# trevordblack/Physically_Based_Renderer

Hardware: AMD Instinct MI355X
Metric: shaded pixels/sec (Mpix/s) + achieved HBM GB/s, 4K G-buffer, 64 lights (higher is better)
Workload: dtype f32

## Files before the change

physically_based_renderer_amd/csrc/pbr_balanced.h:

```cpp
#pragma once
#include <cstdint>
#include <type_traits>

#include "pbr_device_math.h"
#include "pbr_device_math_x2.h"
#include "shade_kernels.h"

namespace pbr {

constexpr int kBalRec = 7;

#ifndef PBR_BAL_PROFILE
#define PBR_BAL_PROFILE 0
#endif
#if PBR_BAL_PROFILE
__device__ unsigned long long* g_bal_prof_buf;
#define BAL_PROF_T(v) const long long v = (long long)__builtin_amdgcn_s_memtime()
#define BAL_PROF_ADD(slot_, val_) do { if ((threadIdx.x & 63) == 0) bal_prof[slot_] += (unsigned long long)(val_); } while (0)
#else
#define BAL_PROF_T(v)
#define BAL_PROF_ADD(i, x)
#endif

constexpr int kBalLdsStride = kBalMaxLights + 4;
// ... 357 lines not shown
                    lz = lds_lights[2 * kBalLdsStride + lane_id];
        const float b0 = ((fabsf(lx - cx) + fabsf(ly - cy)) + fabsf(lz - cz)) + slack;
        const float fr = ((fabsf(lx) + fabsf(ly)) + fabsf(lz)) + pmax;
        bj = (b0 + 0.125f * fr) * (1.0f + 0x1p-20f);
        const float fx = fmaxf(fabsf(lx - mnx), fabsf(lx - mxx)), fy = fmaxf(fabsf(ly - mny), fabsf(ly - mxy)),
                    fz = fmaxf(fabsf(lz - mnz), fabsf(lz - mxz));
        const float gx = fmaxf(fmaxf(mnx - lx, lx - mxx), 0.0f), gy = fmaxf(fmaxf(mny - ly, ly - mxy), 0.0f),
                    gz = fmaxf(fmaxf(mnz - lz, lz - mxz), 0.0f);
        near = (fx * fx + fy * fy) + fz * fz <= 99.9f * 99.9f;
        far = (gx * gx + gy * gy) + gz * gz >= 100.1f * 100.1f;
        close = !((gx * gx + gy * gy) + gz * gz >= (1.02f * dist_lo) * (1.02f * dist_lo));
    }
    const float bmax = bal_wave_max<F>(bj);
    const uint64_t far_m = lanes(far), cross_m = lanes(!near && !far), close_m = lanes(close);
    const v2 cn = v2{0x1p-18f * ((fabsf(n.x.x) + fabsf(n.y.x)) + fabsf(n.z.x)),
                     0x1p-18f * ((fabsf(n.x.y) + fabsf(n.y.y)) + fabsf(n.z.y))};
    const v2 nd = -vfma(n.z, pos.z, vfma(n.y, pos.y, n.x * pos.x));
    const v2 kb = vfma(cn, splat(bmax), nd);
    uint32_t a0 = 0, a1 = 0, c0 = 0, c1 = 0;
    typedef __attribute__((address_space(3))) const float lds_float;
    const uint32_t lbase = (uint32_t)(uintptr_t)(const lds_float*)lds_lights;
    auto word = [&](int qbase, uint32_t& ma, uint32_t& mb) {
        for (int k = 6; k >= 0; k -= 2) {
            const uint32_t la = lbase + 16u * (uint32_t)(qbase + k);
            float4 x1, y1, z1, x0, y0, z0;
            asm volatile(
                "ds_read_b128 %0, %6 offset:16\n\t"
                "ds_read_b128 %1, %6 offset:288\n\t"
                "ds_read_b128 %2, %6 offset:560\n\t"
                "ds_read_b128 %3, %6\n\t"
                "ds_read_b128 %4, %6 offset:272\n\t"
                "ds_read_b128 %5, %6 offset:544\n\t"
                "s_waitcnt lgkmcnt(0)"
                : "=&v"(x1), "=&v"(y1), "=&v"(z1), "=&v"(x0), "=&v"(y0), "=&v"(z0)
                : "v"(la)
                : "memory");
            push_skip_bits4(ma, mb, x1, y1, z1, n, kb);
            push_skip_bits4(ma, mb, x0, y0, z0, n, kb);
        }
    };
    const int n0 = nl < 32 ? nl : 32;
    if (nl > 32) word(8, a1, c1);
    word(0, a0, c0);
    const int n1 = nl - n0;
    const uint32_t k0 = (n0 == 32 ? ~0u : (1u << n0) - 1u) & ~(uint32_t)far_m,
                   k1 = (n1 == 32 ? ~0u : (1u << n1) - 1u) & ~(uint32_t)(far_m >> 32);
    a0 = live_a ? ~a0 & k0 : 0u;
    c0 = live_b ? ~c0 & k0 : 0u;
    a1 = live_a ? ~a1 & k1 : 0u;
    c1 = live_b ? ~c1 & k1 : 0u;
    for (uint64_t cm = cross_m; cm != 0; cm &= cm - 1) {
        const int j = __builtin_ctzll(cm);
        const m2 out = beyond_range(pos, lds_lights[j], lds_lights[kBalLdsStride + j], lds_lights[2 * kBalLdsStride + j]);
        const uint32_t bit = 1u << (j & 31);
        const uint32_t oa = on(out.x) ? bit : 0u, ob = on(out.y) ? bit : 0u;
        if (j < 32) {
            a0 &= ~oa;
            c0 &= ~ob;
        } else {
            a1 &= ~oa;
            c1 &= ~ob;
        }
    }
    bool near_a = false, near_b = false;
    for (uint64_t cm = close_m; cm != 0; cm &= cm - 1) {
        const int j = __builtin_ctzll(cm);
        const f3x2 l = f3x2{splat(lds_lights[j]) - pos.x, splat(lds_lights[kBalLdsStride + j]) - pos.y,
                            splat(lds_lights[2 * kBalLdsStride + j]) - pos.z};
        const m2 ok = ge(sqrt_nr(dot3(l, l)), dist_lo);
        const uint32_t bit = 1u << (j & 31);
        near_a = near_a || (((j < 32 ? a0 : a1) & bit) != 0 && !on(ok.x));
        near_b = near_b || (((j < 32 ? c0 : c1) & bit) != 0 && !on(ok.y));
    }

    BAL_PROF_T(t1);
    BAL_PROF_ADD(0, t1 - t0);
    return BalMasks{a0, a1, c0, c1, near_a, near_b};
}

__device__ __forceinline__ int wave_live_items(const BalMasks& bm) {
    return wave_sum_dpp((__popc(bm.a0) + __popc(bm.a1)) + (__popc(bm.c0) + __popc(bm.c1)));
}


template <bool EXACT>
__device__ __forceinline__ void lighting_balanced_points(const PixelInvariants2& q, const Faithful2& fi,
                                                         const f3x2& pos, bool live_a, bool live_b, BalMasks bm,
                                                         BalancedWaveLds& w, const float* lds_lights, f3x2& sum,
                                                         m2& redo, unsigned long long* bal_prof = nullptr) {
    const int lane_id = (int)(threadIdx.x & 63);
    const uint32_t a0 = bm.a0, a1 = bm.a1, c0 = bm.c0, c1 = bm.c1;
    redo |= mask2(bm.near_a, bm.near_b);
    constexpr int R = EXACT ? kBalRecX : kBalRec;
    BAL_PROF_T(t1);
    PBR_PHASE("rank");

    const int cnt_a = __popc(a0) + __popc(a1), cnt_b = __popc(c0) + __popc(c1);
    w.hist[lane_id] = 0;
    wave_lds_sync();
    const int bin_a = cnt_a < 63 ? cnt_a : 63, bin_b = cnt_b < 63 ? cnt_b : 63;
    const int pos_a = atomicAdd(&w.hist[bin_a], 1);
    const int pos_b = atomicAdd(&w.hist[bin_b], 1);
    wave_lds_sync();
    const int h = w.hist[lane_id];
    const int incl = wave_scan_add_dpp(h);
    wave_lds_sync();
    w.hist[lane_id] = incl - h;
    wave_lds_sync();
    const int rank_a = w.hist[bin_a] + pos_a, rank_b = w.hist[bin_b] + pos_b;
    wave_lds_sync();
    w.rank[lane_id] = make_int2(rank_a, rank_b);
    using Item = std::conditional_t<EXACT, ItemPixelX, ItemPixel>;
    Item ia, ib;
    if constexpr (EXACT) {
        ia = item_pixel_x(q, pos, 0, a0, a1, 2 * lane_id);
        ib = item_pixel_x(q, pos, 1, c0, c1, 2 * lane_id + 1);
    } else {
        ia = item_pixel(q, fi, pos, 0, a0, a1, 2 * lane_id);
        ib = item_pixel(q, fi, pos, 1, c0, c1, 2 * lane_id + 1);
    }
    if (rank_a < 64) store_item(&w.rec[R * rank_a], ia);
    if (rank_b < 64) store_item(&w.rec[R * rank_b], ib);
    wave_lds_sync();
    Item cur = load_item_any<EXACT>(&w.rec[R * lane_id]);
    wave_lds_sync();
    if (rank_a >= 64) store_item(&w.rec[R * (127 - rank_a)], ia);
    if (rank_b >= 64) store_item(&w.rec[R * (127 - rank_b)], ib);
    wave_lds_sync();

    BAL_PROF_T(t2);
    PBR_PHASE("pass2");
    f3x2 acc = splat3(0.0f, 0.0f, 0.0f);
    f3 accx = mk3(0.0f, 0.0f, 0.0f);
    uint64_t fail = 0, second = 0;
    uint64_t m = ((uint64_t)cur.live1 << 32) | cur.live0;
    auto result = [&]() {
        const f3 r = EXACT ? accx : mk3(acc.x.x + acc.x.y, acc.y.x + acc.y.y, acc.z.x + acc.z.y);
        return make_float4(r.x, r.y, r.z, on(fail) ? 0.0f : 1.0f);
    };
    const uint32_t slot_addr = lds_addr(&w.rec[R * lane_id]);
    auto put_result = [&](int k, float4 v) {
        if (k == 0) {
            lds_write2<0>(slot_addr, v.x, v.y);
            lds_write2<2>(slot_addr, v.z, v.w);
        } else {
            lds_write2<4>(slot_addr, v.x, v.y);
            lds_write2<6>(slot_addr, v.z, v.w);
        }
    };
    auto next_pixel = [&]() {
        cur = load_item_any<EXACT>(&w.rec[R * lane_id]);
        m = ((uint64_t)cur.live1 << 32) | cur.live0;
        put_result(0, result());
        acc = splat3(0.0f, 0.0f, 0.0f);
        accx = mk3(0.0f, 0.0f, 0.0f);
    };
    uint64_t zero = lanes(m == 0);
    if (zero != 0) {
        if (on(zero)) next_pixel();
        second = zero;
        const uint64_t first_done = zero;
        zero = lanes(m == 0);
        const uint64_t empty = first_done & zero;
        if (empty != 0 && on(empty)) put_result(1, result());
    }
#if PBR_BAL_PROFILE
    int iters = 0;
#endif
    {
        const uint64_t exec = __builtin_amdgcn_read_exec();
        uint64_t live = ~zero & exec;
        while (live != 0) {
// ... 63 lines not shown
```

physically_based_renderer_amd/csrc/shade_kernels.hip:

```cpp
#include <hip/hip_runtime.h>

#include <cstdint>
#include <type_traits>
#include <vector>

#include "pbr_device_math.h"
#include "pbr_device_math_x2.h"
#include "pbr_balanced.h"
#include "shade_kernels.h"

namespace pbr {

#ifndef PBR_WAVE_TIMELINE
#define PBR_WAVE_TIMELINE 0
#endif
#if PBR_WAVE_TIMELINE
constexpr int kTlWords = 8;
static __device__ unsigned long long* g_wave_tl;
static __device__ long long g_wave_tl_cap;
#define TL_RT(i_) (tl[i_] = (unsigned long long)__builtin_amdgcn_s_memrealtime())
#define TL_BEGIN()                                                                                           \
    unsigned long long tl[kTlWords];                                                                         \
    TL_RT(1);                                                                                                \
    tl[6] = (unsigned long long)__builtin_amdgcn_s_memtime();                                                \
// ... 120 lines not shown
        off += (w < wave) ? c : 0;
        total += c;
    }
    if (keep) {
        const int slot = off + before;
        s.light[3 * slot + 0] = l0;
        s.light[3 * slot + 1] = l1;
        s.light[3 * slot + 2] = l2;
    }
    return total;
}

struct LightRec {
    float4 s, d, p;
};
__device__ __forceinline__ LightRec light_rec(const float4* __restrict__ lights, int j, const PassArgs& ps) {
    j = PBR_BOUNDS(j, ps.n_dir + ps.n_point + ps.n_spot, kBoundsLight);
    return LightRec{lights[3 * j], lights[3 * j + 1], lights[3 * j + 2]};
}
__device__ __forceinline__ m2 light_flag(const LightRec& r) {
    const uint64_t m = (__float_as_uint(r.p.w) << 1) != 0u ? ~0ull : 0ull;
    return m2{m, m};
}
__device__ __forceinline__ float uniform_f(float x) {
    return __builtin_bit_cast(float, __builtin_amdgcn_readfirstlane(__builtin_bit_cast(int, x)));
}

__device__ __forceinline__ bool light_survives(float4 lp, const TileBounds& wb) {
    const float dx = hmax(hmax(wb.mn[0] - lp.x, lp.x - wb.mx[0]), 0.0f);
    const float dy = hmax(hmax(wb.mn[1] - lp.y, lp.y - wb.mx[1]), 0.0f);
    const float dz = hmax(hmax(wb.mn[2] - lp.z, lp.z - wb.mx[2]), 0.0f);
    return (dx * dx + dy * dy + dz * dz) <= kCullRadius * kCullRadius;
}

__device__ __forceinline__ void survivor_masks(const float4* __restrict__ lights, int base, int b1,
                                               const TileBounds& wb, bool cull_enabled, uint64_t (&m)[4]) {
    const int lane = (int)(threadIdx.x & 63);
    float4 lp[4];
#pragma unroll
    for (int k = 0; k < 4; ++k) {
        const int j = base + 64 * k + lane;
        lp[k] = j < b1 && cull_enabled ? lights[3 * j + 2] : make_float4(0.0f, 0.0f, 0.0f, 0.0f);
    }
#pragma unroll
    for (int k = 0; k < 4; ++k) {
        const int j = base + 64 * k + lane;
        m[k] = lanes(j < b1 && (!cull_enabled || light_survives(lp[k], wb)));
    }
}

struct FirstSurvivors {
    uint64_t m[4];
    bool valid = false;
};
__device__ __forceinline__ int wave_light_terms(const float4* __restrict__ lights, const PassArgs& ps,
                                                const TileBounds& wb, bool cull_enabled,
                                                FirstSurvivors* first = nullptr) {
    const int b0 = ps.n_dir, b1 = ps.n_dir + ps.n_point + ps.n_spot;
    if (!cull_enabled) return b1;
    int total = ps.n_dir;
    for (int base = b0; base < b1; base += 256) {
        uint64_t m[4];
        if (first != nullptr && first->valid && base == b0) {
            for (int k = 0; k < 4; ++k) m[k] = first->m[k];
        } else {
            survivor_masks(lights, base, b1, wb, true, m);
            if (first != nullptr && base == b0 && ps.n_spot == 0) {
                for (int k = 0; k < 4; ++k) first->m[k] = m[k];
                first->valid = true;
            }
        }
        total += __popcll(m[0]) + __popcll(m[1]) + __popcll(m[2]) + __popcll(m[3]);
    }
    return total;
}

template <bool CULL, bool LEAN, bool FAITHFUL = false, bool BALANCED = false>
__device__ __forceinline__ f3x2 lighting_fast(const PixelInvariants2& q, const f3x2& pos, m2 fast_ok,
                                              const float4* __restrict__ lights, const PassArgs& ps,
                                              const TileBounds& wb, bool cull_enabled, m2& redo, int& kept_total,
                                              BalancedWaveLds* bal = nullptr, const float* bal_lights = nullptr,
                                              bool geo_a = false, bool geo_b = false, BalMasks bm = BalMasks{},
                                              unsigned long long* bal_prof = nullptr,
                                              const FirstSurvivors* first = nullptr) {
    f3x2 direct = splat3(0.0f, 0.0f, 0.0f);
    Faithful2 fi{};
    if (FAITHFUL) fi = make_faithful<!CULL>(q);
    const int n_dir = BALANCED && !FAITHFUL ? 0 : ps.n_dir;
    for (int j = 0; j < n_dir; ++j) {
        PBR_COLD("directional");
        const LightRec r = light_rec(lights, j, ps);
        m2 ok = fast_ok & light_flag(r);
        if (FAITHFUL) {
            directional_faithful_x2<LEAN, !CULL>(q, fi, r.s, r.d, ok, direct);
        } else {
            const f3x2 c = directional_x2<LEAN>(q, r.s, r.d, ok);
            direct = add3(direct, c);
        }
        redo |= ~ok;
    }
    const int pt_begin = ps.n_dir, sp_begin = ps.n_dir + ps.n_point, end = sp_begin + ps.n_spot;
    auto run_kind = [&](auto spot_tag, int b0, int b1) {
        constexpr bool SPOT = decltype(spot_tag)::value;
        auto point = [&](int j) {
            const LightRec r = light_rec(lights, j, ps);
            m2 ok = fast_ok & light_flag(r);
            if (FAITHFUL) {
                point_or_spot_faithful_x2<SPOT, LEAN, !CULL>(q, fi, pos, r.s, r.d, r.p, ok, direct);
            } else {
                const f3x2 c = point_or_spot_x2<SPOT, LEAN>(q, pos, r.s, r.d, r.p, ok);
                direct = add3(direct, c);
            }
            redo |= ~ok;
        };
        if (!CULL) {
            for (int j = b0; j < b1; ++j) point(j);
            return;
        }
        for (int base = b0; base < b1; base += 256) {
            uint64_t ms[4];
            if (!SPOT && first != nullptr && first->valid && base == b0) {
                for (int k = 0; k < 4; ++k) ms[k] = first->m[k];
            } else {
                survivor_masks(lights, base, b1, wb, cull_enabled, ms);
            }
#pragma unroll
            for (int k = 0; k < 4; ++k) {
                uint64_t m = ms[k];
                kept_total += __popcll(m);
                while (m) {
                    const int jl = base + 64 * k + __builtin_ctzll(m);
                    m &= m - 1;
                    point(jl);
                }
            }
        }
    };
    if (BALANCED)
        lighting_balanced_points<!FAITHFUL>(q, fi, pos, geo_a, geo_b, bm, *bal, bal_lights, direct, redo, bal_prof);
    else
        run_kind(std::false_type{}, pt_begin, sp_begin);
    if (!BALANCED && end > sp_begin) run_kind(std::true_type{}, sp_begin, end);
    if (FAITHFUL) {
        const m2 in_x = eq(direct.x, 0.0f) | (ge(direct.x, 0x1p-100f) & le(direct.x, 0x1p100f));
        const m2 in_y = eq(direct.y, 0.0f) | (ge(direct.y, 0x1p-100f) & le(direct.y, 0x1p100f));
        const m2 in_z = eq(direct.z, 0.0f) | (ge(direct.z, 0x1p-100f) & le(direct.z, 0x1p100f));
        redo |= ~(in_x & in_y & in_z);
    }
    return direct;
}

template <bool CULL>
__device__ __forceinline__ void lighting_exact(const PixelInvariants& qa, const PixelInvariants& qb, f3 pa, f3 pb,
                                               bool need_a, bool need_b, const float4* __restrict__ lights,
                                               const PassArgs& ps, Lds& s, const TileBounds& tb,
                                               bool cull_enabled, f3& da, f3& db) {
    da = mk3(0.0f, 0.0f, 0.0f);
    db = mk3(0.0f, 0.0f, 0.0f);
    bool unused = true;
    for (int base = 0; base < ps.n_dir; base += kChunk) {
        const int cnt = min(kChunk, ps.n_dir - base);
        __syncthreads();
        stage_chunk<false>(lights, base, cnt, s, tb, false, true);
        __syncthreads();
        for (int j = 0; j < cnt; ++j) {
            const float4* r = &s.light[3 * j];
            if (need_a) da = add3(da, directional_light<false>(qa, r[0], r[1], unused));
            if (need_b) db = add3(db, directional_light<false>(qb, r[0], r[1], unused));
        }
    }
    const int pt_begin = ps.n_dir, sp_begin = ps.n_dir + ps.n_point, end = sp_begin + ps.n_spot;
#pragma unroll 1
    for (int kind = 1; kind <= 2; ++kind) {
        const int b0 = kind == 1 ? pt_begin : sp_begin, b1 = kind == 1 ? sp_begin : end;
        for (int base = b0; base < b1; base += kChunk) {
            const int cnt = min(kChunk, b1 - base);
            __syncthreads();
            const int kept = stage_chunk<CULL>(lights, base, cnt, s, tb, cull_enabled, false);
            __syncthreads();
            for (int j = 0; j < kept; ++j) {
                const float4* r = &s.light[3 * j];
                f3 c;
                if (need_a) {
                    const bool lit = kind == 1 ? point_or_spot_light<false, false>(qa, pa, r[0], r[1], r[2], c, unused)
                                               : point_or_spot_light<true, false>(qa, pa, r[0], r[1], r[2], c, unused);
                    if (lit) da = add3(da, c);
                }
                if (need_b) {
                    const bool lit = kind == 1 ? point_or_spot_light<false, false>(qb, pb, r[0], r[1], r[2], c, unused)
                                               : point_or_spot_light<true, false>(qb, pb, r[0], r[1], r[2], c, unused);
                    if (lit) db = add3(db, c);
                }
            }
        }
    }
}

__device__ __forceinline__ void lighting_exact_wave(const PixelInvariants& qa, const PixelInvariants& qb, f3 pa,
                                                    f3 pb, bool need_a, bool need_b, const float4* __restrict__ lights,
                                                    const PassArgs& ps, f3& da, f3& db) {
    da = mk3(0.0f, 0.0f, 0.0f);
    db = mk3(0.0f, 0.0f, 0.0f);
    bool unused = true;
    for (int j = 0; j < ps.n_dir; ++j) {
        const LightRec r = light_rec(lights, j, ps);
        if (need_a) da = add3(da, directional_light<false>(qa, r.s, r.d, unused));
        if (need_b) db = add3(db, directional_light<false>(qb, r.s, r.d, unused));
    }
    const int pt_begin = ps.n_dir, sp_begin = ps.n_dir + ps.n_point, end = sp_begin + ps.n_spot;
    for (int j = pt_begin; j < end; ++j) {
        const LightRec r = light_rec(lights, j, ps);
        const bool spot = j >= sp_begin;
        f3 c;
        if (need_a) {
            const bool lit = spot ? point_or_spot_light<true, false>(qa, pa, r.s, r.d, r.p, c, unused)
                                  : point_or_spot_light<false, false>(qa, pa, r.s, r.d, r.p, c, unused);
            if (lit) da = add3(da, c);
        }
        if (need_b) {
            const bool lit = spot ? point_or_spot_light<true, false>(qb, pb, r.s, r.d, r.p, c, unused)
                                  : point_or_spot_light<false, false>(qb, pb, r.s, r.d, r.p, c, unused);
            if (lit) db = add3(db, c);
// ... 293 lines not shown
            }
        }
        const int cnt = min(64, n - base);
        for (int k = 0; k < cnt; ++k) {
            sum.x = sum.x + __builtin_bit_cast(float, __builtin_amdgcn_readlane(__builtin_bit_cast(int, t.x), k));
            sum.y = sum.y + __builtin_bit_cast(float, __builtin_amdgcn_readlane(__builtin_bit_cast(int, t.y), k));
            sum.z = sum.z + __builtin_bit_cast(float, __builtin_amdgcn_readlane(__builtin_bit_cast(int, t.z), k));
        }
    }
    return sum;
}

template <int AMBIENT, bool F0_PLANE, bool APPLY_AO, bool LANES>
__device__ __forceinline__ float4 shade_pixel_exact(const GBufferArgs& gb, const PassArgs& ps,
                                                    const float4* __restrict__ lights, const float4* __restrict__ env,
                                                    int64_t idx, bool need, bool faithful_finish) {
    if (!LANES) idx = need ? idx : 0;
    idx = PBR_BOUNDS_PIXEL(idx, gb.width, gb.height, gb.row_stride, 1, kBoundsGBuffer);
    const f3 pos = mk3(gb.plane[0][idx], gb.plane[1][idx], gb.plane[2][idx]);
    const f3 n = mk3(gb.plane[3][idx], gb.plane[4][idx], gb.plane[5][idx]);
    const f3 albedo = mk3(gb.plane[6][idx], gb.plane[7][idx], gb.plane[8][idx]);
    const float metallic = gb.plane[9][idx], roughness = gb.plane[10][idx];
    const float ao = APPLY_AO ? gb.plane[11][idx] : 1.0f;
    const f3 f0 = F0_PLANE ? mk3(gb.plane[12][idx], gb.plane[13][idx], gb.plane[14][idx])
                           : mk3(ps.fresnel_r0[0] + metallic * (albedo.x - ps.fresnel_r0[0]),
                                 ps.fresnel_r0[1] + metallic * (albedo.y - ps.fresnel_r0[1]),
                                 ps.fresnel_r0[2] + metallic * (albedo.z - ps.fresnel_r0[2]));
    const f3 eye = mk3(ps.eye[0], ps.eye[1], ps.eye[2]);
    const PixelInvariants q = make_invariants(n, normalize3(sub3(eye, pos)), albedo, f0, metallic, roughness);
    f3 d, unused;
    if (LANES)
        d = lighting_exact_lanes(q, pos, lights, ps);
    else
        lighting_exact_wave(q, q, pos, pos, need, false, lights, ps, d, unused);
    return finish_pixel<AMBIENT, APPLY_AO>(q, ao, d, ps, env, false, faithful_finish);
}

constexpr int kLanesRepassMax = 8;

template <int AMBIENT, bool F0_PLANE, bool APPLY_AO>
__device__ __forceinline__ void repass_exact(const GBufferArgs& gb, const PassArgs& ps,
                                             const float4* __restrict__ lights, const float4* __restrict__ env,
                                             const FrameArgs& fr, int tile_x, int tile_y, int wave_id, bool need_a,
                                             bool need_b, int n_exact, bool faithful) {
    const int tid = threadIdx.x & 63;
    if (n_exact <= kLanesRepassMax) {
        uint64_t ma = lanes(need_a), mb = lanes(need_b);
        while ((ma | mb) != 0) {
            const bool second = ma == 0;
            uint64_t& m = second ? mb : ma;
            const int l = __builtin_ctzll(m);
            m &= m - 1;
            const int rx = tile_x * kTileW + 2 * (l & 31) + (second ? 1 : 0);
            const int ry = tile_y * kTileH + 2 * wave_id + (l >> 5);
            float4 c = shade_pixel_exact<AMBIENT, F0_PLANE, APPLY_AO, true>(gb, ps, lights, env,
                                                                            (int64_t)ry * gb.row_stride + rx, true,
                                                                            faithful);
            if (tid == 0 && alpha_keep(gb, (int64_t)ry * gb.row_stride + rx, c))
                store_pixel(fr, (int64_t)ry * fr.out_stride + rx, c);
        }
    } else {
        const int ln = lane_id_fresh();
        const int rx = tile_x * kTileW + 2 * (ln & 31);
        const int ry = tile_y * kTileH + 2 * wave_id + (ln >> 5);
        const int64_t gi = (int64_t)ry * gb.row_stride + rx, oi = (int64_t)ry * fr.out_stride + rx;
        if (lanes(need_a) != 0) {
            float4 c = shade_pixel_exact<AMBIENT, F0_PLANE, APPLY_AO, false>(gb, ps, lights, env, gi, need_a, faithful);
            if (need_a && alpha_keep(gb, gi, c)) store_pixel(fr, oi, c);
        }
        if (lanes(need_b) != 0) {
            float4 c = shade_pixel_exact<AMBIENT, F0_PLANE, APPLY_AO, false>(gb, ps, lights, env, gi + 1, need_b,
                                                                             faithful);
            if (need_b && alpha_keep(gb, gi + 1, c)) store_pixel(fr, oi + 1, c);
        }
    }
}

template <int AMBIENT, bool F0_PLANE, bool APPLY_AO, bool CULL, int BAL = 0>
__global__ __launch_bounds__(BAL != 0 && PBR_BAL_WAVES == 1 ? 64 : kBlock, PBR_X2_MIN_WAVES) void shade_tile_kernel(
    GBufferArgs gb, PassArgs ps, const float4* __restrict__ lights, const float4* __restrict__ env, FrameArgs fr,
    int32_t* __restrict__ tile_kept, bool exact_only) {
    constexpr bool kOneWave = BAL != 0 && PBR_BAL_WAVES == 1;
    __shared__ std::conditional_t<kOneWave, LdsBal1, Lds> s;
    TL_BEGIN();
    PBR_PHASE("entry");
#if PBR_BAL_PROFILE
    const long long t_entry = (long long)__builtin_amdgcn_s_memtime();
    unsigned long long* bal_prof = s.prof[__builtin_amdgcn_readfirstlane(threadIdx.x) >> 6];
    if ((threadIdx.x & 63) < 16) bal_prof[threadIdx.x & 63] = 0;
#endif
    load_libm_tables<AMBIENT == kAmbientIblDiffuse, (BAL != 0 && PBR_BAL_WAVES == 1 ? 64 : kBlock)>();
    if constexpr (BAL != 0)
        stage_balanced_lights<kOneWave ? 64 : kBlock>(lights, ps.n_dir, ps.n_dir + ps.n_point, s.bal_light,
                                                      BAL == 2 ? 4.0f : 1.0f);
    __syncthreads();
    PBR_PHASE("load_window");

    const int wave_id = kOneWave ? (int)(blockIdx.y & 3) : __builtin_amdgcn_readfirstlane((int)threadIdx.x) >> 6;
    const int wslot = kOneWave ? 0 : wave_id;
    const int tile_y = kOneWave ? (int)(blockIdx.y >> 2) : (int)blockIdx.y;
    const int tid = kOneWave ? 64 * wave_id + (int)threadIdx.x : (int)threadIdx.x;
    const int xa = blockIdx.x * kTileW + 2 * (tid & 31);
    const int y = tile_y * kTileH + (tid >> 5);
    const bool va = (xa < gb.width) && (y < gb.height);
    const bool vb = (xa + 1 < gb.width) && (y < gb.height);
    const int64_t row = (int64_t)y * gb.row_stride;
    const bool ga = va && is_geometry(fr, xa, y), gb_ = vb && is_geometry(fr, xa + 1, y);
    const bool wave_geometry = lanes(ga || gb_) != 0;

    PairIn p = load_pair<F0_PLANE, APPLY_AO>(gb, ps, va ? row + xa : 0, vb ? row + xa + 1 : 0,
                                             vb && gb.pairs_aligned);
    const f3 pa = lane(p.pos, 0), pb = lane(p.pos, 1);

    const bool ok_a = !exact_only && ps.eye_ok && fast_window_ok(pa, lane(p.n, 0), lane(p.albedo, 0), lane(p.f0, 0),
                                                    p.metallic.x, p.roughness.x);
    const bool ok_b = !exact_only && ps.eye_ok && fast_window_ok(pb, lane(p.n, 1), lane(p.albedo, 1), lane(p.f0, 1),
                                                    p.metallic.y, p.roughness.y);
    const m2 fast2 = mask2(ok_a, ok_b);
    TL_LOADED();

    PixelInvariants2 q2;
    if constexpr (BAL == 0) q2 = pair_invariants(p, ps, fast2);
    auto form_q2 = [&]() {
        if constexpr (BAL != 0) q2 = pair_invariants(p, ps, fast2);
    };

    TileBounds wb{};
    bool cull_enabled = false;
    if (CULL) {
        const bool finite = (!ga || (isfinite(pa.x) && isfinite(pa.y) && isfinite(pa.z))) &&
                            (!gb_ || (isfinite(pb.x) && isfinite(pb.y) && isfinite(pb.z)));
        const float big = 3.0e38f;
        wb.mn[0] = uniform_f(wave_min(fminf(ga ? pa.x : big, gb_ ? pb.x : big)));
        wb.mn[1] = uniform_f(wave_min(fminf(ga ? pa.y : big, gb_ ? pb.y : big)));
        wb.mn[2] = uniform_f(wave_min(fminf(ga ? pa.z : big, gb_ ? pb.z : big)));
        wb.mx[0] = uniform_f(wave_max(fmaxf(ga ? pa.x : -big, gb_ ? pb.x : -big)));
        wb.mx[1] = uniform_f(wave_max(fmaxf(ga ? pa.y : -big, gb_ ? pb.y : -big)));
        wb.mx[2] = uniform_f(wave_max(fmaxf(ga ? pa.z : -big, gb_ ? pb.z : -big)));
        cull_enabled = lanes(!finite) == 0;
    }

    int kept_total = 0;
    int bal_items = -1;
    m2 redo = m2{0, 0};
    f3x2 pos2 = p.pos;
    f3x2 d2 = splat3(0.0f, 0.0f, 0.0f);
    bool faithful_wave = false;
    TL_RT(3);
    if (wave_geometry) {
        const v2 nn = dot3(p.n, p.n);
        const bool lean_lane = ok_a && ok_b && nn.x <= 1.0f + 0x1p-20f && nn.y <= 1.0f + 0x1p-20f &&
                               f0_nonzero(lane(p.f0, 0)) && f0_nonzero(lane(p.f0, 1));
        const bool faithful_lane =
            ps.faithful && ok_a && ok_b && p.albedo.x.x >= 0.0f && p.albedo.y.x >= 0.0f && p.albedo.z.x >= 0.0f &&
            p.albedo.x.y >= 0.0f && p.albedo.y.y >= 0.0f && p.albedo.z.y >= 0.0f && p.f0.x.x <= 1.0f &&
            p.f0.y.x <= 1.0f && p.f0.z.x <= 1.0f && p.f0.x.y <= 1.0f && p.f0.y.y <= 1.0f && p.f0.z.y <= 1.0f &&
            p.f0.x.x >= 0.0f && p.f0.y.x >= 0.0f && p.f0.z.x >= 0.0f && p.f0.x.y >= 0.0f && p.f0.y.y >= 0.0f &&
            p.f0.z.y >= 0.0f;
        faithful_wave = BAL != 2 && ps.faithful && lanes(!faithful_lane) == 0;
        if (CULL && faithful_wave && ps.faithful == 2)
            faithful_wave = wave_light_terms(lights, ps, wb, cull_enabled) <= kFaithfulMaxTerms;
        const bool lean_wave = lanes(!lean_lane) == 0;
        if (faithful_wave && lean_wave) {
            if constexpr (BAL == 1 && !CULL) {
#if PBR_BAL_PROFILE
                BAL_PROF_ADD(7, (long long)__builtin_amdgcn_s_memtime() - t_entry);
                unsigned long long* prof = s.prof[wslot];
#else
                unsigned long long* prof = nullptr;
#endif
                PBR_PHASE("pass1");
                const BalMasks bm = balanced_pass1<false>(p.pos, p.n, ga, gb_, ps.n_point, kBalDistLoFaithful, s.bal[wslot],
                                                   s.bal_light, prof);
                bal_items = wave_live_items(bm);
                PBR_PHASE("invariants");
                launder(p);
                q2 = pair_invariants(p, ps, fast2);
                faithful_scale(q2);
                d2 = lighting_fast<false, true, true, true>(q2, p.pos, fast2, lights, ps, wb, cull_enabled, redo,
                                                            kept_total, &s.bal[wslot], s.bal_light, ga, gb_, bm,
                                                            prof);
#if PBR_BAL_PROFILE
                const long long t_l1 = (long long)__builtin_amdgcn_s_memtime();
#endif
                PBR_PHASE("invariants2");
                launder(p);
                q2 = pair_finish_invariants(p, ps, fast2);
                pos2 = p.pos;
#if PBR_BAL_PROFILE
                const v2 dep = dot3(q2.n, q2.v);
                if (dep.x == 12345.0f) pos2.x.x = 0.5f;
                BAL_PROF_ADD(8, (long long)__builtin_amdgcn_s_memtime() - t_l1);
#endif
            } else {
                form_q2();
                if (!CULL) faithful_scale(q2);
#if PBR_BAL_PROFILE
                const long long t_u0 = (long long)__builtin_amdgcn_s_memtime();
                BAL_PROF_ADD(11, t_u0 - t_entry);
                BAL_PROF_ADD(13, 1);
#endif
                d2 = lighting_fast<CULL, true, true>(q2, pos2, fast2, lights, ps, wb, cull_enabled, redo, kept_total);
                if (!CULL) faithful_unscale(q2);
#if PBR_BAL_PROFILE
                const v2 dep = d2.x + d2.y;
                if (dep.x == 12345.0f) pos2.x.x = 0.5f;
                BAL_PROF_ADD(12, (long long)__builtin_amdgcn_s_memtime() - t_u0);
#endif
            }
        } else if (faithful_wave) {
            PBR_COLD("faithful_nonlean");
            form_q2();
            if (!CULL) faithful_scale(q2);
            d2 = lighting_fast<CULL, false, true>(q2, pos2, fast2, lights, ps, wb, cull_enabled, redo, kept_total);
            if (!CULL) faithful_unscale(q2);
        } else if (lean_wave) {
            PBR_PHASE("xpass1");
            if constexpr (BAL == 2 && !CULL) {
#if PBR_BAL_PROFILE
                unsigned long long* prof = s.prof[wslot];
#else
                unsigned long long* prof = nullptr;
#endif
                auto reload = [&]() {
                    asm volatile("" ::: "memory");
                    const int rl = lane_id_fresh();
                    const int rx = blockIdx.x * kTileW + 2 * (rl & 31);
                    const int ry = tile_y * kTileH + 2 * wave_id + (rl >> 5);
                    const int64_t rrow = (int64_t)ry * gb.row_stride + rx;
                    p = load_pair<F0_PLANE, APPLY_AO>(gb, ps, va ? rrow : 0, vb ? rrow + 1 : 0,
                                                      vb && gb.pairs_aligned);
                };
                const BalMasks bm = balanced_pass1<true>(p.pos, p.n, ga, gb_, ps.n_point, kBalDistLoExact, s.bal[wslot],
                                                   s.bal_light, prof);
                bal_items = wave_live_items(bm);
                PBR_PHASE("xinvariants");
                q2 = pair_invariants(p, ps, fast2);
                d2 = lighting_fast<false, true, false, true>(q2, p.pos, fast2, lights, ps, wb, cull_enabled, redo,
                                                             kept_total, &s.bal[wslot], s.bal_light, ga, gb_, bm,
                                                             prof);
                PBR_PHASE("xinvariants2");
                reload();
                q2 = pair_invariants(p, ps, fast2);
                pos2 = p.pos;
            } else {
                form_q2();
                d2 = lighting_fast<CULL, true>(q2, pos2, fast2, lights, ps, wb, cull_enabled, redo, kept_total);
            }
        } else {
            PBR_COLD("general");
            form_q2();
            d2 = lighting_fast<CULL, false>(q2, pos2, fast2, lights, ps, wb, cull_enabled, redo, kept_total);
        }
    } else {
        PBR_COLD("background");
        form_q2();
    }
    TL_RT(4);
    const PixelInvariants ua = unpack_invariants(q2, 0), ub = unpack_invariants(q2, 1);
    f3 da = lane(d2, 0), db = lane(d2, 1);
    const bool need_a = ga && on(redo.x), need_b = gb_ && on(redo.y);
    PBR_PHASE("stats_repass");
    const int n_exact = __popcll(lanes(need_a)) + __popcll(lanes(need_b));
    const int geo_px = __popcll(lanes(ga)) + __popcll(lanes(gb_));
// ... 619 lines not shown
```

Measured before the change: 10500.

## Split heavy pixel light lists into units shared across lanes in balanced pass

Adds a split variant of the balanced point-light loop for the faithful non-exact path. Pixels are ranked by survivor count, and pairs of lights from the heaviest pixels are handed out as work units to lightly loaded lanes. Each lane processes its own item, then a second item, then donated units, and writes partial sums to LDS. The owner lanes then reduce these sums, and failure bits are tracked per item. The goal is to cut wave divergence from uneven per-pixel light counts, at the cost of extra LDS traffic, syncs, bookkeeping and register pressure.

Result: no change. 10610, median of 6 (+1.0%).

```diff
diff --git a/physically_based_renderer_amd/csrc/pbr_balanced.h b/physically_based_renderer_amd/csrc/pbr_balanced.h
--- a/physically_based_renderer_amd/csrc/pbr_balanced.h
+++ b/physically_based_renderer_amd/csrc/pbr_balanced.h
@@ -463,12 +463,230 @@
     return wave_sum_dpp((__popc(bm.a0) + __popc(bm.a1)) + (__popc(bm.c0) + __popc(bm.c1)));
 }
 
+constexpr int kBalUnitCap = 64;
+constexpr int kBalUnitsPerLane = 6;
+constexpr int kBalResFloats = 3 * 128 + 4;
+static_assert(kBalUnitCap <= 64 && 4 * (kBalUnitsPerLane - 1) + 3 <= 23, "unit table and partial-sum layout");
+
+__device__ __forceinline__ void lighting_balanced_points_split(const PixelInvariants2& q, const Faithful2& fi,
+                                                               const f3x2& pos, bool live_a, bool live_b, BalMasks bm,
+                                                               BalancedWaveLds& w, float* res, const float* lds_lights,
+                                                               f3x2& sum, m2& redo,
+                                                               unsigned long long* bal_prof = nullptr) {
+    const int lane_id = (int)(threadIdx.x & 63);
+    const uint32_t a0 = bm.a0, a1 = bm.a1, c0 = bm.c0, c1 = bm.c1;
+    redo |= mask2(bm.near_a, bm.near_b);
+    constexpr int R = kBalRec;
+    uint32_t* const tab = reinterpret_cast<uint32_t*>(w.rank);
+    uint32_t* const recw = reinterpret_cast<uint32_t*>(w.rec);
+    uint32_t* const failed = reinterpret_cast<uint32_t*>(res + 3 * 128);
+    BAL_PROF_T(t1);
+    PBR_PHASE("rank");
+
+    const int cnt_a = __popc(a0) + __popc(a1), cnt_b = __popc(c0) + __popc(c1);
+    reinterpret_cast<uint4*>(recw)[lane_id] = make_uint4(0u, 0u, 0u, 0u);
+    wave_lds_sync();
+    const int bin_a = cnt_a < 63 ? cnt_a : 63, bin_b = cnt_b < 63 ? cnt_b : 63;
+    const int pix_w = lane_id >> 4;
+    const uint32_t pix_a = 1u << ((2 * lane_id) & 31);
+    atomicOr(&recw[4 * bin_a + pix_w], pix_a);
+    atomicOr(&recw[4 * bin_b + pix_w], pix_a << 1);
+    wave_lds_sync();
+    const uint4 hm = reinterpret_cast<const uint4*>(recw)[lane_id];
+    const int h = (__popc(hm.x) + __popc(hm.y)) + (__popc(hm.z) + __popc(hm.w));
+    const int incl = wave_scan_add_dpp(h);
+    w.hist[lane_id] = incl - h;
+    wave_lds_sync();
+    auto place = [&](const uint4 mk, uint32_t below) {
+        const uint32_t own = pix_w == 0 ? mk.x : pix_w == 1 ? mk.y : pix_w == 2 ? mk.z : mk.w;
+        return ((__popc(own & below) + (pix_w > 0 ? __popc(mk.x) : 0)) +
+                ((pix_w > 1 ? __popc(mk.y) : 0) + (pix_w > 2 ? __popc(mk.z) : 0)));
+    };
+    const uint4 ma = reinterpret_cast<const uint4*>(recw)[bin_a], mb = reinterpret_cast<const uint4*>(recw)[bin_b];
+    const int rank_a = w.hist[bin_a] + place(ma, pix_a - 1u), rank_b = w.hist[bin_b] + place(mb, 2u * pix_a - 1u);
+    tab[64 + lane_id] = (uint32_t)(rank_a | (rank_b << 8));
+    wave_lds_sync();
+    const ItemPixel ia = item_pixel(q, fi, pos, 0, a0, a1, 2 * lane_id);
+    const ItemPixel ib = item_pixel(q, fi, pos, 1, c0, c1, 2 * lane_id + 1);
+    if (rank_a < 64) store_item(&w.rec[R * rank_a], ia);
+    if (rank_b < 64) store_item(&w.rec[R * rank_b], ib);
+    wave_lds_sync();
+    ItemPixel cur = load_item(&w.rec[R * lane_id]);
+    wave_lds_sync();
+    if (rank_a >= 64) store_item(&w.rec[R * (127 - rank_a)], ia);
+    if (rank_b >= 64) store_item(&w.rec[R * (127 - rank_b)], ib);
+    wave_lds_sync();
+
+    uint32_t* const own = recw + 4 * R * lane_id;
+    int d_first, d;
+    {
+        uint64_t ms = ((uint64_t)own[24] << 32) | own[23];
+        const int k1 = (__popc(cur.live0) + __popc(cur.live1) + 1) >> 1, k2 = (__popcll(ms) + 1) >> 1;
+        const int t = k1 + k2;
+        const int quota = (wave_sum_dpp(t) + 63) >> 6;
+        const int g0 = min(max(t - quota, 0), k2), d0 = min(max(quota - t, 0), kBalUnitsPerLane);
+        const int gi = wave_scan_add_dpp(g0), di = wave_scan_add_dpp(d0);
+        const int units = min(min(__builtin_amdgcn_readlane(gi, 63), __builtin_amdgcn_readlane(di, 63)), kBalUnitCap);
+        const int g_first = gi - g0;
+        const int g = min(max(units - g_first, 0), g0);
+        d_first = di - d0;
+        d = min(max(units - d_first, 0), d0);
+        if (lane_id < 4) failed[lane_id] = 0u;
+        own[26] = g > 0 ? (uint32_t)(g_first | (g << 8)) : 0u;
+        if (d == 0) d_first = 0;
+        if (g > 0) {
+            const uint32_t hi = (uint32_t)(R * lane_id) << 16;
+            for (int u = g_first; u < g_first + g; ++u) {
+                const int jl = __builtin_ctzll(ms);
+                ms &= ms - 1;
+                const int jh = ms != 0 ? __builtin_ctzll(ms) : jl;
+                ms &= ms - 1;
+                tab[PBR_BOUNDS(u, kBalUnitCap, kBoundsLds)] = (uint32_t)(jl | (jh << 6)) | hi;
+            }
+            own[23] = (uint32_t)ms;
+            own[24] = (uint32_t)(ms >> 32);
+        }
+    }
+    wave_lds_sync();
+
+    BAL_PROF_T(t2);
+    PBR_PHASE("pass2");
+    f3x2 acc = splat3(0.0f, 0.0f, 0.0f);
+    uint64_t fail = 0, second = 0;
+    uint64_t m = ((uint64_t)cur.live1 << 32) | cur.live0;
+    const uint32_t rec_addr = lds_addr(recw), res_addr = lds_addr(res);
+    uint32_t dst = res_addr + 12u * (uint32_t)lane_id;
+    uint32_t useq = (uint32_t)d_first | ((uint32_t)d << 16);
+    uint32_t nw = 0;
+    auto hand_back = [&]() {
+        lds_write2<0>(dst, acc.x.x + acc.x.y, acc.y.x + acc.y.y);
+        lds_write1<2>(dst, acc.z.x + acc.z.y);
+    };
+    auto to_second = [&]() {
+        cur = load_item(&w.rec[R * lane_id]);
+        m = ((uint64_t)cur.live1 << 32) | cur.live0;
+        hand_back();
+        dst = res_addr + 12u * (uint32_t)(64 + lane_id);
+        nw = tab[PBR_BOUNDS((int)(useq & 0xffffu), 128, kBoundsLds)];
+        acc = splat3(0.0f, 0.0f, 0.0f);
+    };
+    auto next_unit = [&]() {
+        hand_back();
+        if (useq >= 0x10000u) {
+            const uint32_t word = nw;
+            const int ti = PBR_BOUNDS((int)(useq & 0xffffu), kBalUnitCap, kBoundsLds);
+            cur = load_item(&w.rec[PBR_BOUNDS((int)(word >> 16), 63 * R + 1, kBoundsLds)]);
+            m = (1ull << (word & 63u)) | (1ull << ((word >> 6) & 63u));
+            useq -= 0x10000u;
+            const uint32_t place = 4u * (uint32_t)(R * lane_id) + 4u * (useq >> 16);
+            tab[ti] = (word & 0xffff0000u) | place;
+            dst = rec_addr + 4u * (uint32_t)PBR_BOUNDS((int)place, 4 * R * 64 - 2, kBoundsLds);
+            useq += 1u;
+            nw = tab[ti + 1];
+            acc = splat3(0.0f, 0.0f, 0.0f);
+        }
+    };
+    uint64_t zero;
+    auto finish_segments = [&](uint64_t done) {
+        if ((fail & done) != 0) {
+            if (on(fail & done)) {
+                int r = on(second) ? 127 - lane_id : lane_id;
+                if (on(second) && dst != res_addr + 12u * (uint32_t)(64 + lane_id))
+                    r = 127 - (int)(tab[PBR_BOUNDS((int)(useq & 0xffffu) - 1, kBalUnitCap, kBoundsLds)] >> 16) / R;
+                atomicOr(&failed[r >> 5], 1u << (r & 31));
+            }
+            fail &= ~done;
+        }
+        const uint64_t first_done = done & ~second, later_done = done & second;
+        if (first_done != 0 && on(first_done)) to_second();
+        if (later_done != 0 && on(later_done)) next_unit();
+        second |= first_done;
+        zero = lanes(m == 0);
+    };
+    zero = lanes(m == 0);
+    if (zero != 0) {
+        const uint64_t first_empty = zero;
+        finish_segments(first_empty);
+        if ((first_empty & zero) != 0) finish_segments(first_empty & zero);
+    }
+#if PBR_BAL_PROFILE
+    int iters = 0;
+#endif
+    {
+        const uint64_t exec = __builtin_amdgcn_read_exec();
+        uint64_t live = ~zero & exec;
+        while (live != 0) {
+#if PBR_BAL_PROFILE
+            ++iters;
+#endif
+            const int j0 = m != 0 ? __builtin_ctzll(m) : kBalMaxLights;
+            m &= m - 1;
+            const int j1 = m != 0 ? __builtin_ctzll(m) : kBalMaxLights;
+            m &= m - 1;
+            m2 oki = m2{~0ull, ~0ull};
+            f3x2 lp, ls;
+            read_pair_lights(lds_lights, j0, j1, lp, ls);
+            faithful_point_items2(cur, lp, ls, oki, acc, live);
+            fail |= ~(oki.x & oki.y) & live;
+            zero = lanes(m == 0);
+            const uint64_t done = zero & live;
+            if (done != 0) finish_segments(done);
+            live = ~zero & exec;
+        }
+    }
+    BAL_PROF_T(t3);
+    PBR_PHASE("handback");
+    wave_lds_sync();
+    {
+        const uint32_t gg = own[26];
+        const int u0 = (int)(gg & 0xffu), u1 = u0 + (int)(gg >> 8);
+        if (u1 > u0) {
+            float* r = res + 3 * (64 + lane_id);
+            float x = r[0], y = r[1], z = r[2];
+            for (int u = u0; u < u1; ++u) {
+                const uint32_t e = tab[PBR_BOUNDS(u, kBalUnitCap, kBoundsLds)];
+                const float* p = reinterpret_cast<const float*>(recw) +
+                                 PBR_BOUNDS((int)(e & 0xffffu), 4 * R * 64 - 2, kBoundsLds);
+                x += p[0];
+                y += p[1];
+                z += p[2];
+            }
+            r[0] = x;
+            r[1] = y;
+            r[2] = z;
+        }
+    }
+    wave_lds_sync();
+    const uint32_t rk = tab[64 + lane_id];
+    const int ra = PBR_BOUNDS((int)(rk & 0xffu), 128, kBoundsLds), rb = PBR_BOUNDS((int)(rk >> 8), 128, kBoundsLds);
+    const float* pa = res + 3 * (ra < 64 ? ra : 191 - ra);
+    const float* pb = res + 3 * (rb < 64 ? rb : 191 - rb);
+    const v2 rx = v2{pa[0], pb[0]}, ry = v2{pa[1], pb[1]}, rz = v2{pa[2], pb[2]};
+    const bool fa = ((failed[ra >> 5] >> (ra & 31)) & 1u) != 0;
+    const bool fb = ((failed[rb >> 5] >> (rb & 31)) & 1u) != 0;
+    wave_lds_sync();
+    sum = f3x2{sum.x + rx, sum.y + ry, sum.z + rz};
+    redo |= mask2(live_a && fa, live_b && fb);
+#if PBR_BAL_PROFILE
+    BAL_PROF_T(t4);
+    BAL_PROF_ADD(1, t2 - t1);
+    BAL_PROF_ADD(2, t3 - t2);
+    BAL_PROF_ADD(3, t4 - t3);
+    BAL_PROF_ADD(4, 1);
+    BAL_PROF_ADD(5, iters);
+#endif
+}
 
 template <bool EXACT>
 __device__ __forceinline__ void lighting_balanced_points(const PixelInvariants2& q, const Faithful2& fi,
                                                          const f3x2& pos, bool live_a, bool live_b, BalMasks bm,
                                                          BalancedWaveLds& w, const float* lds_lights, f3x2& sum,
-                                                         m2& redo, unsigned long long* bal_prof = nullptr) {
+                                                         m2& redo, unsigned long long* bal_prof = nullptr,
+                                                         float* split_res = nullptr) {
+    if constexpr (!EXACT) {
+        lighting_balanced_points_split(q, fi, pos, live_a, live_b, bm, w, split_res, lds_lights, sum, redo, bal_prof);
+        return;
+    }
     const int lane_id = (int)(threadIdx.x & 63);
     const uint32_t a0 = bm.a0, a1 = bm.a1, c0 = bm.c0, c1 = bm.c1;
     redo |= mask2(bm.near_a, bm.near_b);
diff --git a/physically_based_renderer_amd/csrc/shade_kernels.hip b/physically_based_renderer_amd/csrc/shade_kernels.hip
--- a/physically_based_renderer_amd/csrc/shade_kernels.hip
+++ b/physically_based_renderer_amd/csrc/shade_kernels.hip
@@ -226,7 +226,7 @@
                                               BalancedWaveLds* bal = nullptr, const float* bal_lights = nullptr,
                                               bool geo_a = false, bool geo_b = false, BalMasks bm = BalMasks{},
                                               unsigned long long* bal_prof = nullptr,
-                                              const FirstSurvivors* first = nullptr) {
+                                              const FirstSurvivors* first = nullptr, float* bal_res = nullptr) {
     f3x2 direct = splat3(0.0f, 0.0f, 0.0f);
     Faithful2 fi{};
     if (FAITHFUL) fi = make_faithful<!CULL>(q);
@@ -281,7 +281,8 @@
         }
     };
     if (BALANCED)
-        lighting_balanced_points<!FAITHFUL>(q, fi, pos, geo_a, geo_b, bm, *bal, bal_lights, direct, redo, bal_prof);
+        lighting_balanced_points<!FAITHFUL>(q, fi, pos, geo_a, geo_b, bm, *bal, bal_lights, direct, redo, bal_prof,
+                                            bal_res);
     else
         run_kind(std::false_type{}, pt_begin, sp_begin);
     if (!BALANCED && end > sp_begin) run_kind(std::true_type{}, sp_begin, end);
@@ -741,6 +742,7 @@
     int32_t* __restrict__ tile_kept, bool exact_only) {
     constexpr bool kOneWave = BAL != 0 && PBR_BAL_WAVES == 1;
     __shared__ std::conditional_t<kOneWave, LdsBal1, Lds> s;
+    __shared__ float split_res[BAL == 1 && !CULL ? (kOneWave ? 1 : kBlock / 64) : 1][BAL == 1 && !CULL ? kBalResFloats : 1];
     TL_BEGIN();
     PBR_PHASE("entry");
 #if PBR_BAL_PROFILE
@@ -838,7 +840,7 @@
                 faithful_scale(q2);
                 d2 = lighting_fast<false, true, true, true>(q2, p.pos, fast2, lights, ps, wb, cull_enabled, redo,
                                                             kept_total, &s.bal[wslot], s.bal_light, ga, gb_, bm,
-                                                            prof);
+                                                            prof, nullptr, split_res[wslot]);
 #if PBR_BAL_PROFILE
                 const long long t_l1 = (long long)__builtin_amdgcn_s_memtime();
 #endif
```
